# cnuns/Com-MARL

Measured on AMD Instinct MI355X. Metric: env-steps/sec (whole node), PredatorPrey M=10 N=4, 4096 envs at 1/2/4/8 GPUs, higher is better.
Workload: dtype f32

## Files before the change

com-marl_amd/csrc/cm_env_pp10_dev.h:

```cpp
#pragma once
#include "cm_env_dev.h"

namespace cm {
namespace pp10 {

constexpr int S = 10, N = 4, M = 4, D = 21;
constexpr uint32_t ONES = 0x01010101u, HIGH = 0x80808080u, LOW7 = 0x7f7f7f7fu, SIXTEENS = 0x10101010u;

__device__ __forceinline__ uint32_t cell_of(int r, int c) { return (uint32_t)((r + 1) * 16 + c + 1); }
__device__ __forceinline__ int row_of(uint32_t ci) { return (int)(ci >> 4) - 1; }
__device__ __forceinline__ int col_of(uint32_t ci) { return (int)(ci & 15u) - 1; }
__device__ __forceinline__ uint32_t byte_at(uint32_t w, int i) { return (w >> (8 * i)) & 0xffu; }
__device__ __forceinline__ uint32_t set_byte(uint32_t w, int i, uint32_t v) { return (w & ~(0xffu << (8 * i))) | (v << (8 * i)); }
__device__ __forceinline__ uint32_t bcast(uint32_t t) { return t * ONES; }
__device__ __forceinline__ uint32_t any0(uint32_t x) { return (x - ONES) & ~x & HIGH; }
__device__ __forceinline__ uint32_t zero_bytes(uint32_t x) { return ~(((x & LOW7) + LOW7) | x | LOW7); }
__device__ __forceinline__ uint32_t delta_of(int a) { return (uint32_t)(16 * dr_of(a) + dc_of(a)); }
__device__ __forceinline__ int inside(uint32_t t) { return (((t >> 4) - 1u) < 10u) & (((t & 15u) - 1u) < 10u); }
__device__ __forceinline__ int lacks(uint32_t layer, uint32_t t) { return any0(layer ^ bcast(t)) == 0u; }
__device__ __forceinline__ uint32_t live_preys(uint32_t ppos, uint32_t flags) {
    uint32_t w = ppos;
#pragma unroll
    for (int j = 0; j < M; ++j) w |= ((flags >> j) & 1u) ? 0u : (0xffu << (8 * j));
    return w;
// ... 79 lines not shown
        const uint32_t ca = byte_at(apos, sl), cp = byte_at(ppos, sl);
        *at32(p.agent_pos, b * N + sl) = make_int2(row_of(ca), col_of(ca));
        *at32(p.prey_pos, b * M + sl) = make_int2(row_of(cp), col_of(cp));
        *at32(p.alive, b * M + sl) = (uint8_t)((flags >> sl) & 1u);
    }
}

__device__ __forceinline__ void draw_stage(const EnvDev &p, uint32_t rng_step, int32_t act_gid0, uint32_t act_step, uint32_t act_k0,
                                           uint32_t act_k1, int envs, bool all_valid, int buf) {
    const int tx = thread_x(), lane = tx & (WAVE - 1), idx = lane & 15;
    const bool prey = (lane & 16) != 0;
    const uint32_t half = (uint32_t)(lane >> 5);
    const int tgt = (tx >> 6) * 4 + (idx >> 2);
    const int b_raw = blockIdx.x * 16 + tgt;
    const bool valid = all_valid || (tgt < envs && b_raw < p.B);
    const int b = valid ? b_raw : p.B - 1;
    const uint32_t rs = (uint32_t)__shfl((int)rng_step, (idx >> 2) * 16, WAVE);
    uint32_t c0 = prey ? (uint32_t)(p.env_id_offset + b) : (uint32_t)(act_gid0 + b_raw);
    uint32_t c1 = (prey ? rs : act_step) + half;
    uint32_t c2 = prey ? (uint32_t)SITE_PREY : (uint32_t)SITE_ACTION;
    uint32_t c3 = prey ? 2u * (uint32_t)(idx & 3) : (uint32_t)(idx & 3);
    uint32_t k0 = prey ? p.key0 : act_k0, k1 = prey ? p.key1 : act_k1;
#pragma unroll
    for (int r = 0; r < 10; ++r) {
        const uint64_t p0 = (uint64_t)0xD2511F53u * c0, p1 = (uint64_t)0xCD9E8D57u * c2;
        const uint32_t n0 = (uint32_t)(p1 >> 32) ^ c1 ^ k0, n1 = (uint32_t)p1;
        const uint32_t n2 = (uint32_t)(p0 >> 32) ^ c3 ^ k1, n3 = (uint32_t)p0;
        c0 = n0; c1 = n1; c2 = n2; c3 = n3;
        k0 += 0x9E3779B9u; k1 += 0xBB67AE85u;
    }
    *reinterpret_cast<uint4 *>(smem + buf + 16 * lane) = make_uint4(c0, c1, c2, c3);
}

__device__ __forceinline__ void step(const EnvDev &p, State &st, Pre &pre, const Emit em, int act_off, const cm_step_out &out,
                                     const StepOff &off, bool last, int grp, int b_raw, bool grp_live, int lds_base, bool all_valid,
                                     int obs_copy, int draw) {
    Grp<16> g;
    const int tx = thread_x();
    g.sub = (tx & (WAVE - 1)) / 16; g.sl = tx % 16;
    const int sl = g.sl;
    ENV_PROBE(0);
    const bool valid = all_valid || (grp_live && b_raw < p.B);
    const int b = valid ? b_raw : p.B - 1;
    const Rng rng{ (uint32_t)(p.env_id_offset + b), pre.rng_step, p.key0, p.key1 };
    const bool mine = sl < M;
    const uint32_t xw = *reinterpret_cast<const uint32_t *>(smem + draw + 16 * (4 * g.sub + (sl & 3)) + 4 * (sl >> 2));
    const int4 araw = *reinterpret_cast<const int4 *>(smem + act_off);
    const int ain[4] = { araw.x, araw.y, araw.z, araw.w };
    int act[4], bad = 0;
#pragma unroll
    for (int i = 0; i < N; ++i) {
        const int a = ain[i];
        const int bi = (unsigned)a > 4u;
        bad |= bi;
        const int faulty = ((st.flags >> (4 + i)) & 1u) == 0u;
        act[i] = bi ? 4 : ((faulty & (a != 4)) ? 5 : a);
    }
    if (bad && valid) {
        if (sl == 0) raise(p, CM_ERR_ACTION);
        write_back(p, (uint32_t)b, sl, st.apos, st.ppos, st.flags, pre.step_count_in, pre.succ, pre.rng_step);
    }
    const bool commit = valid && !bad;
    ENV_PROBE(1);
    ENV_PROBE(2);

    uint32_t apos = st.apos, ppos = st.ppos, flags = st.flags;
    uint32_t plive = live_preys(ppos, flags);
    int moving = 0;
#pragma unroll
// ... 81 lines not shown
        do_reset<CM_PP, 16>(p, l, rng, cm_rng_tape{}, b, g, done != 0);
        if (done) {
            uint32_t a = 0u, q = 0u;
#pragma unroll
            for (int i = 0; i < N; ++i) { a |= cell_of(AR(l, i), AC(l, i)) << (8 * i); q |= cell_of(PR(l, i), PC(l, i)) << (8 * i); }
            apos = a; ppos = q;
            flags |= 0x0fu;
        }
    }
    if (done) step_count = 0;
    ENV_PROBE(7);
    const float t_clock = done ? pre.t_step0 : pre.t_step;
    plive = live_preys(ppos, flags);
    float vv[6];
    int ci_copy[6];
#pragma unroll
    for (int u = 0; u < 6; ++u) {
        const uint32_t code = ((u < 3 ? em.e0 : em.e1) >> (10 * (u % 3))) & 0x1ffu;
        const uint32_t i = code & 3u, x = code >> 2, w = x & 63u;
        const uint32_t ci = (apos >> (8u * i)) & 0xffu;
        const uint32_t t = ci + w - 17u;
        const int hit = !lacks((x & 64u) ? plive : apos, t);
        const float tab = __shfl(pre.t_rc, x == 36u ? 16 + col_of(ci) : row_of(ci), 64);
        vv[u] = w < 35u ? (hit ? 1.0f : 0.0f) : (x == 37u ? t_clock : tab);
        ci_copy[u] = 16 * u + sl + 3 * (int)i;
    }
    st.apos = apos; st.ppos = ppos; st.flags = (commit && done) ? (flags | 0xf0u) : flags;
    pre.rng_step += 1u;
    if (commit) { pre.step_count_in = step_count; pre.succ = succ; }
    {
        const int sc = pre.step_count_in + 1;
        pre.t_step = p.lut_step[sc <= p.max_steps ? sc : p.max_steps];
    }
    if (!commit) return;
    if (sl == 0) *at32(o.success, off.success + ub) = succ;
    const uint32_t ob = off.obs + ub * (N * D) + (uint32_t)sl;
    float *oc = reinterpret_cast<float *>(smem + obs_copy);
#pragma unroll
    for (int u = 0; u < 6; ++u) {
        if (16 * u + sl < N * D) {
            *at32(o.obs, ob + 16u * u) = vv[u];
            oc[ci_copy[u]] = vv[u];
        }
    }
    static_assert(OBS_COPY_STRIDE == D + 3, "the copy index k + 3i assumes rows of 24 floats");
    if (last) write_back(p, ub, sl, apos, ppos, flags, step_count, succ, rng.step + 1);
    ENV_PROBE(9);
}

}
}
```

com-marl_amd/csrc/cm_policy_w_dev.h:

```cpp
#pragma once
#include <type_traits>

#include "cm_policy_h_dev.h"

namespace cm {
namespace mw {

using mf::FwdArgs;
using mf::v4f;
using mf::fast_tanh;
using mf::EH; using mf::EMB; using mf::H1; using mf::H2; using mf::H3; using mf::MAX_ACT;
using mh::v8h; using mh::v4h; using mh::h16;

constexpr int WG_ENVS = 16, WG_ROWS = 64, KH = 32;
constexpr int FRAG = 64;

struct PackW { int enc1, enc2, attn, gcn, x1, h3, h4, bias, lds_u4, h2, total; };
__host__ __device__ constexpr int frag_u4(int K, int OUT) { return (OUT / 16) * (K / 32) * 2 * FRAG; }
constexpr int BIAS_U4 = 144;
__host__ __device__ constexpr PackW pack_w(int L) {
    PackW o{};
    int off = 0;
    o.enc1 = off; off += frag_u4(KH, EH);
    o.enc2 = off; off += frag_u4(EH, EMB);
// ... 4 lines not shown
    o.h4 = off; off += frag_u4(H3, 32);
    o.bias = off; off += BIAS_U4;
    o.lds_u4 = off;
    o.h2 = off; off += frag_u4(H1, H2);
    o.total = off;
    return o;
}

struct BiasMap { int e1, e2, g, b1, b2, b3, b4, total; };
__host__ __device__ constexpr BiasMap bias_map(int L) {
    BiasMap o{};
    int off = 0;
    o.e1 = off; off += EH; o.e2 = off; off += EMB; o.g = off; off += (L > 0 ? L : 1) * EMB;
    o.b1 = off; off += H1; o.b2 = off; off += H2; o.b3 = off; off += H3; o.b4 = off; off += 32;
    o.total = off;
    return o;
}
__host__ __device__ inline size_t lds_policy_bytes(int L) { return (size_t)pack_w(L).lds_u4 * 16 + WG_ROWS * 4; }
constexpr int DRAW_WAVE_BYTES = 64 * 16;
__host__ __device__ constexpr int draw_lds_off(int L) { return pack_w(L).h3 * 16; }
static_assert((pack_w(1).bias - pack_w(1).h3) * 16 >= (WG_ROWS / 16) * DRAW_WAVE_BYTES, "the draw buffer lies inside the h3 / h4 slots");

struct WeightsW {
    const uint4 *pack;
    int n_act;
};

__host__ __device__ inline int kmap(int q, int g, int e) { return 32 * q + 16 * (e >> 2) + 4 * g + (e & 3); }

template <int KB> struct Act { v8h hi[KB], lo[KB]; };

#define CM_MFW(A, B, ACC) ACC = __builtin_amdgcn_mfma_f32_16x16x32_f16(A, B, ACC, 0, 0, 0)

template <int KB, int CT>
struct Frags {
    v8h h[CT][KB], l[CT][KB];
    template <int TAG = 0>
    __device__ __forceinline__ void fetch(const uint4 *W, int lane) {
#pragma unroll
        for (int ct = 0; ct < CT; ++ct)
#pragma unroll
            for (int q = 0; q < KB; ++q) {
                h[ct][q] = __builtin_bit_cast(v8h, W[((ct * KB + q) * 2 + 0) * FRAG + lane]);
                l[ct][q] = __builtin_bit_cast(v8h, W[((ct * KB + q) * 2 + 1) * FRAG + lane]);
            }
        __builtin_amdgcn_sched_barrier(0);
    }
};

template <int CT, bool ON>
struct BiasR {
    v4f b[ON ? CT : 1];
    template <int C0 = 0>
    __device__ __forceinline__ void fetch(const float *bias, int g) {
        if constexpr (ON) {
#pragma unroll
            for (int ct = C0; ct < CT; ++ct) { const float4 v = *reinterpret_cast<const float4 *>(bias + 16 * ct + 4 * g); b[ct] = (v4f){ v.x, v.y, v.z, v.w }; }
            __builtin_amdgcn_sched_barrier(0);
        }
    }
    __device__ __forceinline__ const v4f *regs() const { return ON ? b : nullptr; }
};
struct NoHook { __device__ __forceinline__ void operator()() const {} };

constexpr float TANH_PRESCALE = 2.8853900817779268f;

template <int N>
__device__ __forceinline__ void tanh_stage(float (&v)[N]) {
    float e[N];
#pragma unroll
    for (int i = 0; i < N; ++i) e[i] = __builtin_amdgcn_exp2f(v[i]);
#pragma unroll
    for (int i = 0; i < N; ++i) e[i] += 1.0f;
#pragma unroll
    for (int i = 0; i < N; ++i) e[i] = __builtin_amdgcn_rcpf(e[i]);
#pragma unroll
    for (int i = 0; i < N; ++i) v[i] = fmaf(-2.0f, e[i], 1.0f);
}
typedef _Float16 v2h __attribute__((ext_vector_type(2)));
typedef float v2f __attribute__((ext_vector_type(2)));
__host__ __device__ inline void split_u(float x, h16 &h, h16 &l) { h = (h16)x; l = (h16)(x - (float)h); }
enum { SPLIT_SUB = 0, SPLIT_MIX = 1, SPLIT_MIXLO = 2 };
constexpr int SPLIT_DEFAULT = SPLIT_MIXLO;
__device__ __forceinline__ float opaque_minus_one() { float m; asm("s_mov_b32 %0, -1.0" : "=s"(m)); return m; }
template <int N, int MODE = SPLIT_DEFAULT>
__device__ __forceinline__ void split_stage(const float (&y)[N], h16 (&h)[N], h16 (&l)[N]) {
    static_assert(N % 2 == 0, "pairs");
    float d[N];
#pragma unroll
    for (int i = 0; i < N; i += 2) { const v2h p = __builtin_convertvector((v2f){ y[i], y[i + 1] }, v2h); h[i] = p[0]; h[i + 1] = p[1]; }
    if constexpr (MODE == SPLIT_MIXLO) {
        const float m1 = opaque_minus_one();
#pragma unroll
        for (int i = 0; i < N; ++i) l[i] = (h16)__builtin_fmaf((float)h[i], m1, y[i]);
        return;
    }
    if constexpr (MODE == SPLIT_MIX) {
        const float m1 = opaque_minus_one();
#pragma unroll
        for (int i = 0; i < N; ++i) d[i] = __builtin_fmaf((float)h[i], m1, y[i]);
    } else {
#pragma unroll
        for (int i = 0; i < N; ++i) d[i] = y[i] - (float)h[i];
    }
#pragma unroll
    for (int i = 0; i < N; i += 2) { const v2h p = __builtin_convertvector((v2f){ d[i], d[i + 1] }, v2h); l[i] = p[0]; l[i + 1] = p[1]; }
}

template <int KB, int CT, bool TANH, bool BIAS, int SPLIT = SPLIT_DEFAULT, int PB0 = CT, class MID = NoHook>
__device__ __forceinline__ void dense_act(const Frags<KB, CT> &f, const float *bias, const Act<KB> &x, Act<CT / 2> &y, v4f *keep, int lane,
                                          float *sv = nullptr, const v4f *pb = nullptr, MID mid = MID{}) {
    const int g = lane >> 4;
    const v4f zero = (v4f){ 0.f, 0.f, 0.f, 0.f };
    v4f acc[CT];
#pragma unroll
    for (int p = 0; p <= CT / 2; ++p) {
        if constexpr (!std::is_same<MID, NoHook>::value) { if (p == CT / 4) mid(); }
        if (p < CT / 2) {
#pragma unroll
            for (int t = 0; t < 2; ++t) {
                const int ct = 2 * p + t;
                if (BIAS && ct >= PB0) acc[ct] = pb[ct];
                else if (BIAS) { const float4 b = *reinterpret_cast<const float4 *>(bias + 16 * ct + 4 * g); acc[ct] = (v4f){ b.x, b.y, b.z, b.w }; }
#pragma unroll
                for (int q = 0; q < KB; ++q) {
                    const v4f a0 = (q == 0 && !BIAS) ? zero : acc[ct];
                    acc[ct] = __builtin_amdgcn_mfma_f32_16x16x32_f16(f.h[ct][q], x.lo[q], a0, 0, 0, 0);
                    acc[ct] = __builtin_amdgcn_mfma_f32_16x16x32_f16(f.l[ct][q], x.hi[q], acc[ct], 0, 0, 0);
                    acc[ct] = __builtin_amdgcn_mfma_f32_16x16x32_f16(f.h[ct][q], x.hi[q], acc[ct], 0, 0, 0);
                }
            }
        }
        if (p > 0) {
            float v[8];
#pragma unroll
            for (int e = 0; e < 8; ++e) v[e] = acc[2 * (p - 1) + (e >> 2)][e & 3];
            if (TANH) tanh_stage<8>(v);
            if (keep) {
#pragma unroll
                for (int e = 0; e < 8; ++e) keep[2 * (p - 1) + (e >> 2)][e & 3] = v[e];
            }
            if (sv) {
                *reinterpret_cast<float4 *>(sv + 16 * (2 * (p - 1)) + 4 * g) = make_float4(v[0], v[1], v[2], v[3]);
                *reinterpret_cast<float4 *>(sv + 16 * (2 * (p - 1) + 1) + 4 * g) = make_float4(v[4], v[5], v[6], v[7]);
            }
            h16 h[8], l[8];
            split_stage<8, SPLIT>(v, h, l);
#pragma unroll
            for (int e = 0; e < 8; ++e) { y.hi[p - 1][e] = h[e]; y.lo[p - 1][e] = l[e]; }
        }
// ... 48 lines not shown
template <bool LEAN = false>
struct ResidentW {
    Frags<4, 4> h2;
    struct None {};
    std::conditional_t<LEAN, Frags<2, 2>, None> h3;
    std::conditional_t<LEAN, Frags<1, 2>, None> h4;
    template <class R, class F>
    static __device__ __forceinline__ const F &pick(const R &resident, const F &own) { if constexpr (LEAN) return resident; else return own; }
    template <int LHOPS>
    __device__ __forceinline__ void fetch(const WeightsW &w, int lane) {
        h2.template fetch<LEAN>(w.pack + pack_w(LHOPS).h2, lane);
        if constexpr (LEAN) {
            h3.template fetch<LEAN>(w.pack + pack_w(LHOPS).h3, lane);
            h4.template fetch<LEAN>(w.pack + pack_w(LHOPS).h4, lane);
#pragma unroll
            for (int ct = 0; ct < 2; ++ct) {
#pragma unroll
                for (int q = 0; q < 2; ++q) { asm volatile("" : "+a"(h3.h[ct][q])); asm volatile("" : "+a"(h3.l[ct][q])); }
                asm volatile("" : "+a"(h4.h[ct][0])); asm volatile("" : "+a"(h4.l[ct][0]));
            }
        }
#pragma unroll
        for (int ct = 0; ct < 4; ++ct)
#pragma unroll
            for (int q = 0; q < 4; ++q) { asm volatile("" : "+a"(h2.h[ct][q])); asm volatile("" : "+a"(h2.l[ct][q])); }
    }
};

struct StepOff { uint32_t actions, probs, attn; };
template <class T>
__device__ __forceinline__ T *at32(T *base, uint32_t elem) { return reinterpret_cast<T *>(reinterpret_cast<char *>(base) + (uint32_t)(elem * (uint32_t)sizeof(T))); }
template <int LHOPS, bool OBS_LDS = false, bool TRAIN = false, int HEADK = 0, bool STEP32 = false, bool LEAN = false>
__device__ __forceinline__ void policy_tile_w(const FwdArgs &a, int n_act, const ResidentW<LEAN> &res, const unsigned char *lds, int blk,
                                              int32_t *act_lds, int obs_row = 0, const StepOff so = StepOff{}, int draw_off = 0) {
    static_assert(!STEP32 || (!TRAIN && HEADK == 0), "step offsets: the acting forward of the rollout");
    static_assert(!LEAN || (!TRAIN && HEADK == 0), "the lean tile: the acting forward of the rollout");
    constexpr int E1H = LEAN ? 4 : 8, E2H = LEAN ? 2 : 4;
    constexpr int PB_H2 = LEAN ? 0 : 4, PB_H3 = LEAN ? 0 : 2;
    static_assert(HEADK == 0 || TRAIN, "the critic head exists as training forward only");
    static_assert(LHOPS >= 1 && LHOPS <= 2, "wave-owned forward: one or two hops");
    const int tid = thread_x(), wave = tid >> 6, lane = tid & 63, c = lane & 15, g = lane >> 4;
    constexpr PackW pk = pack_w(LHOPS);
    constexpr BiasMap bm = bias_map(LHOPS);
    const uint4 *WL = reinterpret_cast<const uint4 *>(lds);
    const float *BL = reinterpret_cast<const float *>(lds + (size_t)pk.bias * 16);
    const int s0 = blk * WG_ENVS;
    const int row = wave * 16 + c;
    const size_t grow = (size_t)s0 * 4 + row;
    const int env_l = wave * 4 + (c >> 2), agent = c & 3;
    const bool diag = g == (c >> 2);
    const bool rv = s0 + env_l < a.S;

    CM_WPROBE(2);
    Act<1> xo;
    {
        float ov[8];
        if constexpr (OBS_LDS) {
            const float4 *src = reinterpret_cast<const float4 *>(lds + obs_row + 32 * (g < 3 ? g : 0));
            const float4 v0 = src[0], v1 = src[1];
            const float vv[8] = { v0.x, v0.y, v0.z, v0.w, v1.x, v1.y, v1.z, v1.w };
#pragma unroll
            for (int e = 0; e < 8; ++e) ov[e] = (rv && g < 3) ? vv[e] : 0.0f;
        } else {
        const float *src = a.obs + (rv ? grow : 0) * a.d;
#pragma unroll
        for (int e = 0; e < 8; ++e) { const int k = 8 * g + e; const float v = src[k < a.d ? k : 0]; ov[e] = (rv && k < a.d) ? v : 0.0f; }
        }
        h16 h[8], l[8];
        split_stage<8>(ov, h, l);
#pragma unroll
        for (int e = 0; e < 8; ++e) { xo.hi[0][e] = h[e]; xo.lo[0][e] = l[e]; }
    }
    uint32_t draw_step = 0u;
    if constexpr (!LEAN) draw_step = a.policy_step + (a.step_base ? *a.step_base : 0u);

    Frags<1, 8> f_e1; f_e1.template fetch<LEAN>(WL + pk.enc1, lane);
    BiasR<8, LEAN> r_e1;
    Frags<4, 4> f_e2;
    if constexpr (!LEAN) f_e2.template fetch<LEAN>(WL + pk.enc2, lane);
    auto sv_row = [&](float *base, int width) -> float * { return (TRAIN && base && rv) ? base + grow * (size_t)width : nullptr; };
    Act<4> a1;
    if constexpr (LEAN)
        dense_act<1, 8, true, true, SPLIT_DEFAULT, E1H>(f_e1, BL + bm.e1, xo, a1, nullptr, lane, nullptr, r_e1.regs(),
                                                        [&] { r_e1.template fetch<E1H>(BL + bm.e1, g); f_e2.template fetch<LEAN>(WL + pk.enc2, lane); });
    else dense_act<1, 8, true, true>(f_e1, BL + bm.e1, xo, a1, nullptr, lane, sv_row(a.sv_a1, EH));
    BiasR<4, LEAN> r_e2;
    Frags<2, 4> f_at;
    if constexpr (!LEAN) f_at.template fetch<LEAN>(WL + pk.attn, lane);
    v4f E[4];
    Act<2> xe;
    if constexpr (LEAN)
        dense_act<4, 4, true, true, SPLIT_DEFAULT, E2H>(f_e2, BL + bm.e2, a1, xe, E, lane, nullptr, r_e2.regs(),
                                                        [&] { r_e2.template fetch<E2H>(BL + bm.e2, g); f_at.template fetch<LEAN>(WL + pk.attn, lane); });
    else dense_act<4, 4, true, true>(f_e2, BL + bm.e2, a1, xe, E, lane, sv_row(a.sv_e, EMB));
    Frags<2, 4> f_g; f_g.template fetch<LEAN>(WL + pk.gcn, lane);
    CM_WPROBE(3);

    float m[4];
    {
        Act<2> xq;
        dense_act<2, 4, false, false>(f_at, nullptr, xe, xq, nullptr, lane, sv_row(a.sv_q, EMB));
        v4f hh = (v4f){ 0.f, 0.f, 0.f, 0.f };
#pragma unroll
        for (int q = 0; q < 2; ++q) { CM_MFW(xe.hi[q], xq.lo[q], hh); CM_MFW(xe.lo[q], xq.hi[q], hh); CM_MFW(xe.hi[q], xq.hi[q], hh); }
        float sc[4], mx = -INFINITY, sum = 0.0f;
#pragma unroll
        for (int r = 0; r < 4; ++r) { sc[r] = hh[r]; mx = fmaxf(mx, sc[r]); }
#pragma unroll
        for (int r = 0; r < 4; ++r) { m[r] = __builtin_amdgcn_exp2f((sc[r] - mx) * 1.4426950408889634f); sum += m[r]; }
        const float rs = __builtin_amdgcn_rcpf(sum);
#pragma unroll
        for (int r = 0; r < 4; ++r) m[r] *= rs;
    }
    const size_t env_g = (size_t)s0 + env_l;
    if (a.attn && diag && rv) {
        float *dst = STEP32 ? at32(a.attn, so.attn + (uint32_t)env_g * 16u + 4u * (uint32_t)agent) : a.attn + env_g * 16 + 4 * agent;
        __builtin_nontemporal_store(m[0], dst); __builtin_nontemporal_store(m[1], dst + 1);
        __builtin_nontemporal_store(m[2], dst + 2); __builtin_nontemporal_store(m[3], dst + 3);
    }

    CM_WPROBE(5);
    Act<2> xh = xe;
    Frags<2, HEADK == 0 ? 8 : 4> f_x1;
    BiasR<8, LEAN> r_b1;
    BiasR<4, LEAN> r_b2;
    BiasR<2, LEAN> r_b3;
    BiasR<2, LEAN> r_b4;
#pragma unroll
    for (int l = 0; l < LHOPS; ++l) {
        v4f hw[4];
        dense_f32<2, 4, true, false>(f_g, nullptr, xh, hw, lane);
        if constexpr (TRAIN) {
            if (a.sv_hw[l] && s0 + wave * 4 + g < a.S) {
                float *dst = a.sv_hw[l] + ((size_t)s0 * 4 + wave * 16 + 4 * g) * EMB + c;
#pragma unroll
                for (int ct = 0; ct < 4; ++ct)
#pragma unroll
                    for (int r = 0; r < 4; ++r) dst[(size_t)r * EMB + 16 * ct] = hw[ct][r] * (1.0f / TANH_PRESCALE);
            }
        }
        BiasR<4, LEAN> r_g; r_g.fetch(BL + bm.g + l * EMB, g);
        if (l + 1 < LHOPS) f_g.template fetch<LEAN>(WL + pk.gcn + (l + 1) * frag_u4(EMB, EMB), lane);
        else {
            r_b1.fetch(BL + bm.b1, g);
            f_x1.template fetch<LEAN>(WL + pk.x1, lane);
        }
        float cf[4], den = 0.0f;
#pragma unroll
        for (int r = 0; r < 4; ++r) {
            float x = m[r];
            if (a.adj && rv) x *= a.adj[env_g * 16 + 4 * agent + r];
            if (a.chan && rv) x *= a.chan[(env_g * LHOPS + l) * 16 + 4 * agent + r];
            cf[r] = x; den += x;
        }
        const float rden = __builtin_amdgcn_rcpf(den + 1e-12f);
        v4h bh, bl;
        {
            float cn[4];
            h16 h[4], lo_[4];
#pragma unroll
            for (int r = 0; r < 4; ++r) cn[r] = diag ? cf[r] * rden : 0.0f;
            split_stage<4>(cn, h, lo_);
#pragma unroll
            for (int r = 0; r < 4; ++r) { bh[r] = h[r]; bl[r] = lo_[r]; }
        }
        const bool last = l == LHOPS - 1;
        v4h ah[4], al[4];
        {
            float hv[16];
            h16 h[16], lo_[16];
#pragma unroll
            for (int i = 0; i < 16; ++i) hv[i] = hw[i >> 2][i & 3];
            split_stage<16>(hv, h, lo_);
#pragma unroll
            for (int i = 0; i < 16; ++i) { ah[i >> 2][i & 3] = h[i]; al[i >> 2][i & 3] = lo_[i]; }
        }
        v4f acc[4];
#pragma unroll
        for (int ct = 0; ct < 4; ++ct) {
            v4f b0;
            if constexpr (LEAN) b0 = r_g.b[ct];
            else { const float4 b = *reinterpret_cast<const float4 *>(BL + bm.g + l * EMB + 16 * ct + 4 * g); b0 = (v4f){ b.x, b.y, b.z, b.w }; }
            acc[ct] = __builtin_amdgcn_mfma_f32_16x16x16f16(ah[ct], bl, b0, 0, 0, 0);
            acc[ct] = __builtin_amdgcn_mfma_f32_16x16x16f16(al[ct], bh, acc[ct], 0, 0, 0);
            acc[ct] = __builtin_amdgcn_mfma_f32_16x16x16f16(ah[ct], bh, acc[ct], 0, 0, 0);
        }
#pragma unroll
        for (int p = 0; p < 2; ++p) {
            float v[8];
#pragma unroll
            for (int e = 0; e < 8; ++e) v[e] = acc[2 * p + (e >> 2)][e & 3];
            tanh_stage<8>(v);
            if (last && !a.no_residual) {
#pragma unroll
                for (int e = 0; e < 8; ++e) v[e] += E[2 * p + (e >> 2)][e & 3];
            }
            if constexpr (TRAIN) {
                if (float *sv = sv_row(a.sv_h[l], EMB)) {
                    *reinterpret_cast<float4 *>(sv + 16 * (2 * p) + 4 * g) = make_float4(v[0], v[1], v[2], v[3]);
                    *reinterpret_cast<float4 *>(sv + 16 * (2 * p + 1) + 4 * g) = make_float4(v[4], v[5], v[6], v[7]);
                }
            }
            h16 h[8], lo_[8];
            split_stage<8>(v, h, lo_);
#pragma unroll
            for (int e = 0; e < 8; ++e) { xh.hi[p][e] = h[e]; xh.lo[p][e] = lo_[e]; }
        }
    }

    CM_WPROBE(6);
    if constexpr (HEADK == 1) {
        Frags<2, 1> f_d2; f_d2.template fetch<LEAN>(WL + pk.h3, lane);
        Act<2> xd;
        dense_act<2, 4, true, true>(f_x1, BL + bm.b1, xh, xd, nullptr, lane, sv_row(a.sv_x1, EMB));
        v4f val[1];
        dense_f32<2, 1, false, true>(f_d2, BL + bm.b2, xd, val, lane);
        float v = (g == 0 && rv) ? val[0][0] : 0.0f;
        if (a.sv_out && g == 0 && rv) a.sv_out[grow] = v;
        v += __shfl_xor(v, 1);
        v += __shfl_xor(v, 2);
        if (a.values && g == 0 && rv && agent == 0) a.values[(size_t)s0 + env_l] = v;
        return;
    } else {
    Act<4> x1;
    if constexpr (LEAN) {
        dense_act<2, 8, true, true, SPLIT_DEFAULT, 0>(f_x1, BL + bm.b1, xh, x1, nullptr, lane, nullptr, r_b1.regs(),
                                                      [&] { r_b2.fetch(BL + bm.b2, g); r_b3.fetch(BL + bm.b3, g); r_b4.fetch(BL + bm.b4, g); });
    } else dense_act<2, 8, true, true>(f_x1, BL + bm.b1, xh, x1, nullptr, lane, sv_row(a.sv_x1, H1));
    Frags<2, 2> f_h3_lds;
    Frags<1, 2> f_h4_lds;
    if constexpr (!LEAN) { f_h3_lds.template fetch<LEAN>(WL + pk.h3, lane); f_h4_lds.template fetch<LEAN>(WL + pk.h4, lane); }
    const Frags<2, 2> &f_h3 = res.pick(res.h3, f_h3_lds);
    const Frags<1, 2> &f_h4 = res.pick(res.h4, f_h4_lds);
    float u = 0.0f;
    if constexpr (!TRAIN && !LEAN) {
        const u32x4 xr = philox4x32_10((uint32_t)(a.env_id_offset + (int)env_g), draw_step, SITE_ACTION, (uint32_t)agent, a.key0, a.key1);
        u = unit_f32(xr.x);
    }
    CM_WPROBE(7);
    Act<2> x2;
    dense_act<4, 4, true, true, SPLIT_DEFAULT, PB_H2>(res.h2, BL + bm.b2, x1, x2, nullptr, lane, sv_row(a.sv_x2, H2), r_b2.regs());
    Act<1> x3;
    dense_act<2, 2, true, true, SPLIT_DEFAULT, PB_H3>(f_h3, BL + bm.b3, x2, x3, nullptr, lane, sv_row(a.sv_x3, H3), r_b3.regs());
    v4f lg[2];
    if constexpr (LEAN) u = unit_f32(*reinterpret_cast<const uint32_t *>(lds + draw_off + 16 * c));
    dense_f32<1, 2, false, true, LEAN>(f_h4, BL + bm.b4, x3, lg, lane, r_b4.regs());

    CM_WPROBE(9);
    const int A = n_act;
    float p[MAX_ACT];
#pragma unroll
    for (int cc = 0; cc < MAX_ACT; ++cc) p[cc] = cc < 4 ? lg[0][cc] : (cc == 4 ? lg[1][0] : 0.0f);
    if constexpr (TRAIN) {
        if (a.sv_out && g == 0 && rv) {
#pragma unroll
            for (int cc = 0; cc < 5; ++cc) if (cc < A) a.sv_out[grow * A + cc] = p[cc];
        }
    }
    float mx = -INFINITY, sum = 0.0f, msum = 0.0f;
#pragma unroll
// ... 57 lines not shown
```

com-marl_amd/csrc/cm_rollout_w_body.h:

```cpp
    static_assert(!COND || (!CARRY && !TAPE && SHAPE == 0), "the conditions twins are the non-carried, tape-less builds");
    static_assert(SHAPE == 0 || CARRY, "shape constants are built into the carried form only");
    if constexpr (SHAPE == 1) {
        p.S = 10; p.M = 4; p.R = 1; p.W = 3; p.d = 21; p.rcp_d = 1.0f / 21.0f; p.rcp_W = 1.0f / 3.0f; p.rcp_WW = 1.0f / 9.0f;
        p.lds_env = lds_env_bytes(10, 4, 4);
        a.N = 4; a.d = 21; a.L = LHOPS;
        a.avail = nullptr; a.greedy = 0; a.adj = nullptr; a.chan = nullptr; a.probe = nullptr;
        __builtin_assume(a.actions != nullptr); __builtin_assume(a.probs != nullptr); __builtin_assume(a.attn != nullptr);
        if constexpr (!PROBES) p.stop = 0;
        a.policy_step += a.step_base ? *a.step_base : 0u;
        a.step_base = nullptr;
    }
    const int n_act = SHAPE == 1 ? 5 : w.n_act;
    static_assert(!CARRY || (PRE && !TAPE), "the carried form is the prefetching, tape-less build");
    const cm_rng_tape tape = TAPE ? tape_arg : cm_rng_tape{};
    if constexpr (!TAPE) p.rng_mode = CM_RNG_PHILOX;
    p.scen = CM_PP; p.N = 4; p.lpe = 16; p.rcp_N = 0.25f; p.rcp_NN = 0.0625f;
    if constexpr (CARRY) { p.adj_const = 1; p.ch_const = 1; p.channel = CM_CH_FC; }
    extern __shared__ __attribute__((aligned(16))) unsigned char lds_w[];
    constexpr int LPE = 16;
    constexpr int ACT_OFF = mw::pack_w(LHOPS).lds_u4 * 16, ENV_BASE = ACT_OFF + mw::WG_ROWS * 4;
    constexpr int DRAW_OFF = mw::draw_lds_off(LHOPS);
    int32_t *act = reinterpret_cast<int32_t *>(lds_w + ACT_OFF);
    const bool probe = PROBES && p.stop == -2 && blockIdx.x == 0 && thread_x() == 0;
    const unsigned long long t_in = probe ? __builtin_amdgcn_s_memtime() : 0ull;
    mw::stage_w<LHOPS, SHAPE == 1>(w, lds_w, thread_x());
    mw::ResidentW<SHAPE == 1> res;
    res.template fetch<LHOPS>(w, thread_x() & 63);
    __syncthreads();
    if (probe) { g_w_probe[3] = __builtin_amdgcn_s_memtime() - t_in; g_w_probe[0] = g_w_probe[1] = g_w_probe[2] = g_w_probe[4] = 0; }
    const int envs = FULLWG ? mw::WG_ENVS : min(mw::WG_ENVS, a.S - (int)blockIdx.x * mw::WG_ENVS);
    EnvPre pre{};
    pp10::State st{};
    pp10::Pre pp{};
    pp10::Emit em{};
    int obs_row = 0, obs_env = -1;
    if constexpr (CARRY) {
        const int tx = thread_x(), grp = tx / LPE, lane = tx & 63, cc = lane & 15;
        const bool live = FULLWG || grp < envs;
        const Lds l0 = make_lds(p.S, p.N, p.M, ENV_BASE + p.lds_env * grp, p.status);
        obs_env = l0.win;
        const int env_l = (tx >> 6) * 4 + (cc >> 2);
        obs_row = make_lds(p.S, p.N, p.M, ENV_BASE + p.lds_env * env_l, p.status).win + (cc & 3) * OBS_COPY_STRIDE * 4;
        float *oc = reinterpret_cast<float *>(lds_w + obs_env);
        const int b0 = blockIdx.x * mw::WG_ENVS + (live ? grp : 0);
        const bool ok = live && b0 < a.S;
        for (int k = tx % LPE; k < 4 * OBS_COPY_STRIDE; k += LPE) {
            const int i = k / OBS_COPY_STRIDE, f = k - i * OBS_COPY_STRIDE;
            oc[k] = (ok && f < a.d) ? a.obs[((size_t)b0 * 4 + i) * a.d + f] : 0.0f;
        }
        if constexpr (SHAPE == 1) {
            const int b = (live && b0 < p.B) ? b0 : p.B - 1;
            st = pp10::load_state(p, b);
            pp = pp10::load_pre(p, b, tx % LPE, tx);
            em = pp10::emit_codes(tx % LPE);
        } else pre = env_prefetch<CM_PP, LPE>(p, b0, live);
    }
    EnvCondVals cv{};
    if constexpr (COND) {
        const int grp = thread_x() / LPE;
        const int b0 = blockIdx.x * mw::WG_ENVS + ((FULLWG || grp < envs) ? grp : 0);
        cv = load_cond(cond, ((FULLWG || grp < envs) && b0 < p.B) ? b0 : p.B - 1);
    }
    for (int t = 0; t < c.n_steps; ++t) {
        asm volatile("" ::: "memory");
        const int tx = thread_x(), grp = tx / LPE;
        const bool live = FULLWG || grp < envs;
        const bool env_wave = FULLWG || (tx & ~63) / LPE < envs;
        const int b_raw = blockIdx.x * mw::WG_ENVS + (live ? grp : 0);
        mf::FwdArgs at = a;
        at.policy_step = a.policy_step + (uint32_t)t;
        const uint32_t ut = (uint32_t)t;
        if constexpr (SHAPE != 1) {
        at.obs = a.obs + (size_t)t * c.obs;
        at.adj = a.adj ? a.adj + (size_t)t * c.dist_adj : nullptr;
        at.chan = a.chan ? a.chan + (size_t)t * c.channels : nullptr;
        at.actions = a.actions ? a.actions + (size_t)t * c.actions : nullptr;
        at.probs = a.probs ? a.probs + (size_t)t * c.probs : nullptr;
        at.attn = a.attn ? a.attn + (size_t)t * c.attn : nullptr;
        }
        const unsigned long long t0 = probe ? __builtin_amdgcn_s_memtime() : 0ull;
        const int draw = DRAW_OFF + __builtin_amdgcn_readfirstlane(tx >> 6) * mw::DRAW_WAVE_BYTES + (t & 1) * (mw::DRAW_WAVE_BYTES / 2);
        if constexpr (SHAPE == 1) {
            if ((t & 1) == 0) pp10::draw_stage(p, pp.rng_step, a.env_id_offset, at.policy_step, a.key0, a.key1, envs, FULLWG, draw);
            asm volatile("" ::: "memory");
        }
        if constexpr (COND) { if constexpr (PRE) pre = env_prefetch<CM_PP, LPE>(apply_cond(p, cv), b_raw, live); }
        else
        if constexpr (PRE && !CARRY) pre = env_prefetch<CM_PP, LPE>(p, b_raw, live);
        if constexpr (SHAPE == 1)
            mw::policy_tile_w<LHOPS, true, false, 0, true, true>(at, n_act, res, lds_w, blockIdx.x, act, obs_row,
                                                           mw::StepOff{ ut * (uint32_t)c.actions, ut * (uint32_t)c.probs, ut * (uint32_t)c.attn }, draw);
        else mw::policy_tile_w<LHOPS, CARRY>(at, n_act, res, lds_w, blockIdx.x, act, obs_row);
        asm volatile("s_waitcnt lgkmcnt(0)" ::: "memory");
        const unsigned long long t1 = probe ? __builtin_amdgcn_s_memtime() : 0ull;
        cm_step_out ot = out;
        if constexpr (SHAPE != 1) {
        if (ot.obs) ot.obs += (size_t)t * c.obs;
        if (ot.reward) ot.reward += (size_t)t * c.reward;
        if (ot.reward_f64) ot.reward_f64 += (size_t)t * c.reward_f64;
        if (ot.done) ot.done += (size_t)t * c.done;
        if (ot.details) ot.details += (size_t)t * c.details;
        if (ot.dist_adj) ot.dist_adj += (size_t)t * c.dist_adj;
        if (ot.channels) ot.channels += (size_t)t * c.channels;
        if (ot.prey_alive) ot.prey_alive += (size_t)t * c.prey_alive;
        if (ot.success) ot.success += (size_t)t * c.success;
        if (ot.path_len) ot.path_len += (size_t)t * c.path_len;
        }
        if (env_wave) {
            const int32_t *my_act = act + (live ? grp : 0) * 4;
            if constexpr (COND) {
                const EnvDev q = apply_cond(p, cv);
                if constexpr (PRE) {
                    const bool bad = env_stage<CM_PP, LPE>(q, pre, my_act, grp, ENV_BASE);
                    env_body<CM_PP, LPE>(q, nullptr, my_act, tape, ot, 0, grp, b_raw, live, ENV_BASE, nullptr, true, pre.rng_step, pre.step_count_in,
                                         pre.succ, pre.t_row, pre.t_col, pre.t_step0, pre.t_step, pre.t_rew, bad, FULLWG);
                } else env_body<CM_PP, LPE>(q, nullptr, my_act, tape, ot, 0, grp, b_raw, live, ENV_BASE);
            } else if constexpr (CARRY && SHAPE == 1) {
                const pp10::StepOff so{ ut * (uint32_t)c.obs, ut * (uint32_t)c.reward, ut * (uint32_t)c.reward_f64, ut * (uint32_t)c.done,
                                        ut * (uint32_t)c.details, ut * (uint32_t)c.prey_alive, ut * (uint32_t)c.success, ut * (uint32_t)c.path_len };
                pp10::step(p, st, pp, em, ACT_OFF + (live ? grp : 0) * 16, ot, so, t == c.n_steps - 1, grp, b_raw, live, ENV_BASE, FULLWG, obs_env, draw + mw::DRAW_WAVE_BYTES / 4);
            } else if constexpr (CARRY) {
                const bool bad = env_stage<CM_PP, LPE>(p, pre, my_act, grp, ENV_BASE);
                EnvCarry carry{ pre.step_count_in, pre.succ, 0 };
                env_body<CM_PP, LPE>(p, nullptr, my_act, tape, ot, 0, grp, b_raw, live, ENV_BASE, nullptr, true, pre.rng_step, pre.step_count_in,
                                     pre.succ, pre.t_row, pre.t_col, pre.t_step0, pre.t_step, pre.t_rew, bad, FULLWG, &carry, obs_env);
                pre = env_pre_carry<CM_PP, LPE>(p, pre, carry, grp, ENV_BASE);
            } else if constexpr (PRE) {
                const bool bad = env_stage<CM_PP, LPE>(p, pre, my_act, grp, ENV_BASE);
                env_body<CM_PP, LPE>(p, nullptr, my_act, tape, ot, 0, grp, b_raw, live, ENV_BASE, nullptr, true, pre.rng_step, pre.step_count_in,
                                     pre.succ, pre.t_row, pre.t_col, pre.t_step0, pre.t_step, pre.t_rew, bad, FULLWG);
            } else env_body<CM_PP, LPE>(p, nullptr, my_act, tape, ot, 0, grp, b_raw, live, ENV_BASE);
        }
        const unsigned long long tf = probe ? __builtin_amdgcn_s_memtime() : 0ull;
        if constexpr (!CARRY) {
            __builtin_amdgcn_fence(__ATOMIC_RELEASE, "workgroup");
            __builtin_amdgcn_fence(__ATOMIC_ACQUIRE, "workgroup");
        }
        if (probe) { const unsigned long long t2 = __builtin_amdgcn_s_memtime(); g_w_probe[0] += 1; g_w_probe[1] += t1 - t0; g_w_probe[2] += t2 - t1; g_w_probe[4] += t2 - tf; }
    }
    if constexpr (CARRY) {
        if (tl.on) {
            const int tx = thread_x(), grp = tx / LPE, sl = tx % LPE;
            const int b0 = blockIdx.x * mw::WG_ENVS + grp;
            if ((FULLWG || grp < envs) && b0 < a.S) {
                const float *oc = reinterpret_cast<const float *>(lds_w + obs_env);
                float *dst = tl.obs_dst + (size_t)b0 * 4 * a.d;
                const float rcp_d = p.rcp_d;
                for (int k = sl; k < 4 * a.d; k += LPE) { const int i = fdiv(k, a.d, rcp_d), f = k - i * a.d; dst[k] = oc[i * OBS_COPY_STRIDE + f]; }
            }
            if ((tx & 63) == 0) {
                const unsigned int last = gridDim.x * (blockDim.x >> 6) - 1;
                if (atomicAdd(tl.ticket, 1u) == last) { *tl.base += (uint32_t)c.n_steps; *tl.ticket = 0u; }
            }
        }
    }
```

Measured before the change: 463.6 million.

## Prefetch next step's encoder weights and biases from LDS during env step

The lean policy forward now loads the first encoder layer's weight fragments and bias registers one step ahead. It issues those LDS reads from inside the environment step, through a hook placed before the observation writes, so their latency overlaps env work. Later layers' weights and biases are read through explicit LDS address-space pointers and pinned with 'landed' barriers, with bias fetches rescheduled into dense_act hooks. The cost is more live registers across the env step, which may add pressure or spills. The env_wave check is also made wave-uniform through readfirstlane.

```diff
diff --git a/com-marl_amd/csrc/cm_env_pp10_dev.h b/com-marl_amd/csrc/cm_env_pp10_dev.h
--- a/com-marl_amd/csrc/cm_env_pp10_dev.h
+++ b/com-marl_amd/csrc/cm_env_pp10_dev.h
@@ -135,9 +135,10 @@
     *reinterpret_cast<uint4 *>(smem + buf + 16 * lane) = make_uint4(c0, c1, c2, c3);
 }
 
+template <class AHEAD>
 __device__ __forceinline__ void step(const EnvDev &p, State &st, Pre &pre, const Emit em, int act_off, const cm_step_out &out,
                                      const StepOff &off, bool last, int grp, int b_raw, bool grp_live, int lds_base, bool all_valid,
-                                     int obs_copy, int draw) {
+                                     int obs_copy, int draw, AHEAD ahead) {
     Grp<16> g;
     const int tx = thread_x();
     g.sub = (tx & (WAVE - 1)) / 16; g.sl = tx % 16;
@@ -285,8 +286,9 @@
         const int sc = pre.step_count_in + 1;
         pre.t_step = p.lut_step[sc <= p.max_steps ? sc : p.max_steps];
     }
+    if (sl == 0 && commit) *at32(o.success, off.success + ub) = succ;
+    ahead();
     if (!commit) return;
-    if (sl == 0) *at32(o.success, off.success + ub) = succ;
     const uint32_t ob = off.obs + ub * (N * D) + (uint32_t)sl;
     float *oc = reinterpret_cast<float *>(smem + obs_copy);
 #pragma unroll
diff --git a/com-marl_amd/csrc/cm_policy_w_dev.h b/com-marl_amd/csrc/cm_policy_w_dev.h
--- a/com-marl_amd/csrc/cm_policy_w_dev.h
+++ b/com-marl_amd/csrc/cm_policy_w_dev.h
@@ -60,6 +60,9 @@
 
 #define CM_MFW(A, B, ACC) ACC = __builtin_amdgcn_mfma_f32_16x16x32_f16(A, B, ACC, 0, 0, 0)
 
+typedef __attribute__((address_space(3))) const v4f *LdsV4;
+__device__ __forceinline__ LdsV4 lds_v4(uint32_t addr) { return (LdsV4)(uintptr_t)addr; }
+
 template <int KB, int CT>
 struct Frags {
     v8h h[CT][KB], l[CT][KB];
@@ -74,22 +77,65 @@
             }
         __builtin_amdgcn_sched_barrier(0);
     }
+    __device__ __forceinline__ void fetch_at(uint32_t addr, int slot) {
+        uint32_t rel = 16u * (uint32_t)slot;
+        if (16 * (slot + CT * KB * 2 * FRAG) > 65536) { addr += rel; rel = 0u; asm("" : "+v"(addr)); }
+#pragma unroll
+        for (int ct = 0; ct < CT; ++ct)
+#pragma unroll
+            for (int q = 0; q < KB; ++q) {
+                h[ct][q] = __builtin_bit_cast(v8h, *lds_v4(addr + rel + 16u * (uint32_t)(((ct * KB + q) * 2 + 0) * FRAG)));
+                l[ct][q] = __builtin_bit_cast(v8h, *lds_v4(addr + rel + 16u * (uint32_t)(((ct * KB + q) * 2 + 1) * FRAG)));
+            }
+        __builtin_amdgcn_sched_barrier(0);
+    }
+    __device__ __forceinline__ void landed() {
+        __builtin_amdgcn_sched_barrier(0);
+        asm volatile("" : "+v"(l[CT - 1][KB - 1]));
+        __builtin_amdgcn_sched_barrier(0);
+    }
 };
 
 template <int CT, bool ON>
 struct BiasR {
     v4f b[ON ? CT : 1];
     template <int C0 = 0>
-    __device__ __forceinline__ void fetch(const float *bias, int g) {
-        if constexpr (ON) {
-#pragma unroll
-            for (int ct = C0; ct < CT; ++ct) { const float4 v = *reinterpret_cast<const float4 *>(bias + 16 * ct + 4 * g); b[ct] = (v4f){ v.x, v.y, v.z, v.w }; }
-            __builtin_amdgcn_sched_barrier(0);
-        }
+    __device__ __forceinline__ void fetch_at(uint32_t addr, int off) {
+#pragma unroll
+        for (int ct = C0; ct < CT; ++ct) b[ct] = *lds_v4(addr + 4u * (uint32_t)(off + 16 * ct));
+        __builtin_amdgcn_sched_barrier(0);
+    }
+    __device__ __forceinline__ void landed() {
+        __builtin_amdgcn_sched_barrier(0);
+        asm volatile("" : "+v"(b[CT - 1]));
+        __builtin_amdgcn_sched_barrier(0);
     }
     __device__ __forceinline__ const v4f *regs() const { return ON ? b : nullptr; }
 };
 struct NoHook { __device__ __forceinline__ void operator()() const {} };
+template <bool ON>
+struct E1Ahead {
+    struct None {};
+    std::conditional_t<ON, BiasR<8, true>, None> r;
+    std::conditional_t<ON, Frags<1, 8>, None> f;
+    uint32_t fa, ba;
+    template <int LHOPS>
+    __device__ __forceinline__ void init(const unsigned char *lds, int lane) {
+        if constexpr (ON) {
+            typedef __attribute__((address_space(3))) const unsigned char *LdsB;
+            fa = (uint32_t)(uintptr_t)(LdsB)(lds + 16 * lane);
+            ba = (uint32_t)(uintptr_t)(LdsB)(lds + (size_t)pack_w(LHOPS).bias * 16 + 16 * (lane >> 4));
+            asm volatile("" : "+v"(fa), "+v"(ba));
+        }
+    }
+    template <int LHOPS>
+    __device__ __forceinline__ void fetch() {
+        if constexpr (ON) {
+            r.fetch_at(ba, bias_map(LHOPS).e1);
+            f.fetch_at(fa, pack_w(LHOPS).enc1);
+        }
+    }
+};
 
 constexpr float TANH_PRESCALE = 2.8853900817779268f;
 
@@ -135,15 +181,16 @@
     for (int i = 0; i < N; i += 2) { const v2h p = __builtin_convertvector((v2f){ d[i], d[i + 1] }, v2h); l[i] = p[0]; l[i + 1] = p[1]; }
 }
 
-template <int KB, int CT, bool TANH, bool BIAS, int SPLIT = SPLIT_DEFAULT, int PB0 = CT, class MID = NoHook>
+template <int KB, int CT, bool TANH, bool BIAS, int SPLIT = SPLIT_DEFAULT, int PB0 = CT, class MID = NoHook, class LATE = NoHook>
 __device__ __forceinline__ void dense_act(const Frags<KB, CT> &f, const float *bias, const Act<KB> &x, Act<CT / 2> &y, v4f *keep, int lane,
-                                          float *sv = nullptr, const v4f *pb = nullptr, MID mid = MID{}) {
+                                          float *sv = nullptr, const v4f *pb = nullptr, MID mid = MID{}, LATE late = LATE{}) {
     const int g = lane >> 4;
     const v4f zero = (v4f){ 0.f, 0.f, 0.f, 0.f };
     v4f acc[CT];
 #pragma unroll
     for (int p = 0; p <= CT / 2; ++p) {
         if constexpr (!std::is_same<MID, NoHook>::value) { if (p == CT / 4) mid(); }
+        if constexpr (!std::is_same<LATE, NoHook>::value) { if (p == CT / 2 - 1) late(); }
         if (p < CT / 2) {
 #pragma unroll
             for (int t = 0; t < 2; ++t) {
@@ -258,10 +305,10 @@
 __device__ __forceinline__ T *at32(T *base, uint32_t elem) { return reinterpret_cast<T *>(reinterpret_cast<char *>(base) + (uint32_t)(elem * (uint32_t)sizeof(T))); }
 template <int LHOPS, bool OBS_LDS = false, bool TRAIN = false, int HEADK = 0, bool STEP32 = false, bool LEAN = false>
 __device__ __forceinline__ void policy_tile_w(const FwdArgs &a, int n_act, const ResidentW<LEAN> &res, const unsigned char *lds, int blk,
-                                              int32_t *act_lds, int obs_row = 0, const StepOff so = StepOff{}, int draw_off = 0) {
+                                              int32_t *act_lds, int obs_row = 0, const StepOff so = StepOff{}, int draw_off = 0, E1Ahead<LEAN> *e1a = nullptr) {
     static_assert(!STEP32 || (!TRAIN && HEADK == 0), "step offsets: the acting forward of the rollout");
     static_assert(!LEAN || (!TRAIN && HEADK == 0), "the lean tile: the acting forward of the rollout");
-    constexpr int E1H = LEAN ? 4 : 8, E2H = LEAN ? 2 : 4;
+    constexpr int E1H = LEAN ? 0 : 8, E2H = LEAN ? 0 : 4;
     constexpr int PB_H2 = LEAN ? 0 : 4, PB_H3 = LEAN ? 0 : 2;
     static_assert(HEADK == 0 || TRAIN, "the critic head exists as training forward only");
     static_assert(LHOPS >= 1 && LHOPS <= 2, "wave-owned forward: one or two hops");
@@ -300,32 +347,39 @@
     uint32_t draw_step = 0u;
     if constexpr (!LEAN) draw_step = a.policy_step + (a.step_base ? *a.step_base : 0u);
 
-    Frags<1, 8> f_e1; f_e1.template fetch<LEAN>(WL + pk.enc1, lane);
-    BiasR<8, LEAN> r_e1;
+    Frags<1, 8> f_e1;
+    if constexpr (!LEAN) f_e1.template fetch<LEAN>(WL + pk.enc1, lane);
     Frags<4, 4> f_e2;
+    BiasR<4, LEAN> r_e2;
     if constexpr (!LEAN) f_e2.template fetch<LEAN>(WL + pk.enc2, lane);
     auto sv_row = [&](float *base, int width) -> float * { return (TRAIN && base && rv) ? base + grow * (size_t)width : nullptr; };
     Act<4> a1;
+    if constexpr (LEAN) e1a->f.landed();
     if constexpr (LEAN)
-        dense_act<1, 8, true, true, SPLIT_DEFAULT, E1H>(f_e1, BL + bm.e1, xo, a1, nullptr, lane, nullptr, r_e1.regs(),
-                                                        [&] { r_e1.template fetch<E1H>(BL + bm.e1, g); f_e2.template fetch<LEAN>(WL + pk.enc2, lane); });
+        dense_act<1, 8, true, true, SPLIT_DEFAULT, E1H>(e1a->f, BL + bm.e1, xo, a1, nullptr, lane, nullptr, e1a->r.regs(),
+                                                        [&] { f_e2.fetch_at(e1a->fa, pk.enc2); }, [&] { r_e2.fetch_at(e1a->ba, bm.e2); });
+    if constexpr (LEAN) r_e2.landed();
     else dense_act<1, 8, true, true>(f_e1, BL + bm.e1, xo, a1, nullptr, lane, sv_row(a.sv_a1, EH));
-    BiasR<4, LEAN> r_e2;
     Frags<2, 4> f_at;
     if constexpr (!LEAN) f_at.template fetch<LEAN>(WL + pk.attn, lane);
     v4f E[4];
     Act<2> xe;
     if constexpr (LEAN)
         dense_act<4, 4, true, true, SPLIT_DEFAULT, E2H>(f_e2, BL + bm.e2, a1, xe, E, lane, nullptr, r_e2.regs(),
-                                                        [&] { r_e2.template fetch<E2H>(BL + bm.e2, g); f_at.template fetch<LEAN>(WL + pk.attn, lane); });
+                                                        [&] { f_at.fetch_at(e1a->fa, pk.attn); });
     else dense_act<4, 4, true, true>(f_e2, BL + bm.e2, a1, xe, E, lane, sv_row(a.sv_e, EMB));
-    Frags<2, 4> f_g; f_g.template fetch<LEAN>(WL + pk.gcn, lane);
+    if constexpr (LEAN) f_at.landed();
+    BiasR<4, LEAN> r_g[LHOPS];
+    Frags<2, 4> f_g;
+    if constexpr (LEAN) { r_g[0].fetch_at(e1a->ba, bm.g); f_g.fetch_at(e1a->fa, pk.gcn); }
+    else f_g.template fetch<LEAN>(WL + pk.gcn, lane);
     CM_WPROBE(3);
 
     float m[4];
     {
         Act<2> xq;
         dense_act<2, 4, false, false>(f_at, nullptr, xe, xq, nullptr, lane, sv_row(a.sv_q, EMB));
+        if constexpr (LEAN) f_g.landed();
         v4f hh = (v4f){ 0.f, 0.f, 0.f, 0.f };
 #pragma unroll
         for (int q = 0; q < 2; ++q) { CM_MFW(xe.hi[q], xq.lo[q], hh); CM_MFW(xe.lo[q], xq.hi[q], hh); CM_MFW(xe.hi[q], xq.hi[q], hh); }
@@ -355,6 +409,7 @@
 #pragma unroll
     for (int l = 0; l < LHOPS; ++l) {
         v4f hw[4];
+        if constexpr (LEAN) { if (l > 0) f_g.landed(); }
         dense_f32<2, 4, true, false>(f_g, nullptr, xh, hw, lane);
         if constexpr (TRAIN) {
             if (a.sv_hw[l] && s0 + wave * 4 + g < a.S) {
@@ -365,11 +420,12 @@
                     for (int r = 0; r < 4; ++r) dst[(size_t)r * EMB + 16 * ct] = hw[ct][r] * (1.0f / TANH_PRESCALE);
             }
         }
-        BiasR<4, LEAN> r_g; r_g.fetch(BL + bm.g + l * EMB, g);
-        if (l + 1 < LHOPS) f_g.template fetch<LEAN>(WL + pk.gcn + (l + 1) * frag_u4(EMB, EMB), lane);
-        else {
-            r_b1.fetch(BL + bm.b1, g);
-            f_x1.template fetch<LEAN>(WL + pk.x1, lane);
+        if constexpr (LEAN) {
+            if (l + 1 < LHOPS) { r_g[l + 1].fetch_at(e1a->ba, bm.g + (l + 1) * EMB); f_g.fetch_at(e1a->fa, pk.gcn + (l + 1) * frag_u4(EMB, EMB)); }
+            else { r_b1.fetch_at(e1a->ba, bm.b1); f_x1.fetch_at(e1a->fa, pk.x1); }
+        } else {
+            if (l + 1 < LHOPS) f_g.template fetch<LEAN>(WL + pk.gcn + (l + 1) * frag_u4(EMB, EMB), lane);
+            else f_x1.template fetch<LEAN>(WL + pk.x1, lane);
         }
         float cf[4], den = 0.0f;
 #pragma unroll
@@ -405,7 +461,7 @@
 #pragma unroll
         for (int ct = 0; ct < 4; ++ct) {
             v4f b0;
-            if constexpr (LEAN) b0 = r_g.b[ct];
+            if constexpr (LEAN) b0 = r_g[l].b[ct];
             else { const float4 b = *reinterpret_cast<const float4 *>(BL + bm.g + l * EMB + 16 * ct + 4 * g); b0 = (v4f){ b.x, b.y, b.z, b.w }; }
             acc[ct] = __builtin_amdgcn_mfma_f32_16x16x16f16(ah[ct], bl, b0, 0, 0, 0);
             acc[ct] = __builtin_amdgcn_mfma_f32_16x16x16f16(al[ct], bh, acc[ct], 0, 0, 0);
@@ -450,8 +506,9 @@
     } else {
     Act<4> x1;
     if constexpr (LEAN) {
+        f_x1.landed();
         dense_act<2, 8, true, true, SPLIT_DEFAULT, 0>(f_x1, BL + bm.b1, xh, x1, nullptr, lane, nullptr, r_b1.regs(),
-                                                      [&] { r_b2.fetch(BL + bm.b2, g); r_b3.fetch(BL + bm.b3, g); r_b4.fetch(BL + bm.b4, g); });
+                                                      [&] { r_b2.fetch_at(e1a->ba, bm.b2); r_b3.fetch_at(e1a->ba, bm.b3); r_b4.fetch_at(e1a->ba, bm.b4); });
     } else dense_act<2, 8, true, true>(f_x1, BL + bm.b1, xh, x1, nullptr, lane, sv_row(a.sv_x1, H1));
     Frags<2, 2> f_h3_lds;
     Frags<1, 2> f_h4_lds;
diff --git a/com-marl_amd/csrc/cm_rollout_w_body.h b/com-marl_amd/csrc/cm_rollout_w_body.h
--- a/com-marl_amd/csrc/cm_rollout_w_body.h
+++ b/com-marl_amd/csrc/cm_rollout_w_body.h
@@ -29,6 +29,8 @@
     __syncthreads();
     if (probe) { g_w_probe[3] = __builtin_amdgcn_s_memtime() - t_in; g_w_probe[0] = g_w_probe[1] = g_w_probe[2] = g_w_probe[4] = 0; }
     const int envs = FULLWG ? mw::WG_ENVS : min(mw::WG_ENVS, a.S - (int)blockIdx.x * mw::WG_ENVS);
+    mw::E1Ahead<SHAPE == 1> e1a;
+    if constexpr (SHAPE == 1) { e1a.template init<LHOPS>(lds_w, thread_x() & 63); e1a.template fetch<LHOPS>(); }
     EnvPre pre{};
     pp10::State st{};
     pp10::Pre pp{};
@@ -65,7 +67,8 @@
         asm volatile("" ::: "memory");
         const int tx = thread_x(), grp = tx / LPE;
         const bool live = FULLWG || grp < envs;
-        const bool env_wave = FULLWG || (tx & ~63) / LPE < envs;
+        bool env_wave = FULLWG || (tx & ~63) / LPE < envs;
+        if constexpr (SHAPE == 1 && !FULLWG) env_wave = __builtin_amdgcn_readfirstlane(tx >> 6) * (64 / LPE) < envs;
         const int b_raw = blockIdx.x * mw::WG_ENVS + (live ? grp : 0);
         mf::FwdArgs at = a;
         at.policy_step = a.policy_step + (uint32_t)t;
@@ -89,7 +92,7 @@
         if constexpr (PRE && !CARRY) pre = env_prefetch<CM_PP, LPE>(p, b_raw, live);
         if constexpr (SHAPE == 1)
             mw::policy_tile_w<LHOPS, true, false, 0, true, true>(at, n_act, res, lds_w, blockIdx.x, act, obs_row,
-                                                           mw::StepOff{ ut * (uint32_t)c.actions, ut * (uint32_t)c.probs, ut * (uint32_t)c.attn }, draw);
+                                                           mw::StepOff{ ut * (uint32_t)c.actions, ut * (uint32_t)c.probs, ut * (uint32_t)c.attn }, draw, &e1a);
         else mw::policy_tile_w<LHOPS, CARRY>(at, n_act, res, lds_w, blockIdx.x, act, obs_row);
         asm volatile("s_waitcnt lgkmcnt(0)" ::: "memory");
         const unsigned long long t1 = probe ? __builtin_amdgcn_s_memtime() : 0ull;
@@ -106,7 +109,7 @@
         if (ot.success) ot.success += (size_t)t * c.success;
         if (ot.path_len) ot.path_len += (size_t)t * c.path_len;
         }
-        if (env_wave) {
+        if (SHAPE == 1 && !FULLWG ? __builtin_expect(env_wave, true) : env_wave) {
             const int32_t *my_act = act + (live ? grp : 0) * 4;
             if constexpr (COND) {
                 const EnvDev q = apply_cond(p, cv);
@@ -118,7 +121,8 @@
             } else if constexpr (CARRY && SHAPE == 1) {
                 const pp10::StepOff so{ ut * (uint32_t)c.obs, ut * (uint32_t)c.reward, ut * (uint32_t)c.reward_f64, ut * (uint32_t)c.done,
                                         ut * (uint32_t)c.details, ut * (uint32_t)c.prey_alive, ut * (uint32_t)c.success, ut * (uint32_t)c.path_len };
-                pp10::step(p, st, pp, em, ACT_OFF + (live ? grp : 0) * 16, ot, so, t == c.n_steps - 1, grp, b_raw, live, ENV_BASE, FULLWG, obs_env, draw + mw::DRAW_WAVE_BYTES / 4);
+                pp10::step(p, st, pp, em, ACT_OFF + (live ? grp : 0) * 16, ot, so, t == c.n_steps - 1, grp, b_raw, live, ENV_BASE, FULLWG, obs_env, draw + mw::DRAW_WAVE_BYTES / 4,
+                           [&] { e1a.template fetch<LHOPS>(); });
             } else if constexpr (CARRY) {
                 const bool bad = env_stage<CM_PP, LPE>(p, pre, my_act, grp, ENV_BASE);
                 EnvCarry carry{ pre.step_count_in, pre.succ, 0 };
@@ -130,7 +134,7 @@
                 env_body<CM_PP, LPE>(p, nullptr, my_act, tape, ot, 0, grp, b_raw, live, ENV_BASE, nullptr, true, pre.rng_step, pre.step_count_in,
                                      pre.succ, pre.t_row, pre.t_col, pre.t_step0, pre.t_step, pre.t_rew, bad, FULLWG);
             } else env_body<CM_PP, LPE>(p, nullptr, my_act, tape, ot, 0, grp, b_raw, live, ENV_BASE);
-        }
+        } else e1a.template fetch<LHOPS>();
         const unsigned long long tf = probe ? __builtin_amdgcn_s_memtime() : 0ull;
         if constexpr (!CARRY) {
             __builtin_amdgcn_fence(__ATOMIC_RELEASE, "workgroup");
```

New measurement: 470.9 million, median of 6. 1.02x the previous value.
